# falfab/orb_slam_cuda

Measured on AMD Instinct MI355X. Metric: frames/s ORB extract+match, 1241×376 mono nFeatures=2000; achieved HBM GB/s, higher is better.
Workload: dtype u8

## Files before the change

orb_slam_cuda_amd/csrc/orbx_host.hip:

```cpp
#include <hip/hip_runtime.h>

#include <algorithm>
#include <atomic>
#include <chrono>
#include <condition_variable>
#include <cfloat>
#include <cstdarg>
#include <climits>
#include <cmath>
#include <cstdio>
#include <cstdlib>
#include <cstring>
#include <mutex>
#include <string>
#include <thread>
#include <vector>

#include "orbx_internal.h"
#include "orbx_sincosf.h"

namespace orbx {

__global__ __launch_bounds__(256) void copy2d_kernel(uint8_t* __restrict__ d, size_t dp, const uint8_t* __restrict__ s,
                                                     size_t sp, size_t w, size_t rows) {
// ... 12 lines not shown
size_t quadtree_lds_bytes(const ExtractParams& P);
size_t quadtree_legacy_lds_bytes(const ExtractParams& P);
size_t quadtree_sorted_lds_bytes(const ExtractParams& P, int big);
int quadtree_sorted_ownmax(const ExtractParams& P, int big, size_t budget);
extern const void* quadtree_kernel_ptr(const ExtractParams& P);
size_t pyr_band_lds_bytes(const ExtractParams& P);
void blur_strip_dims(int small, int* strip, int* rows);
extern const void* pyr_band_kernel_ptr();
extern int pyr_band_occupancy(size_t lds);
}

using namespace orbx;

static size_t out_desc_off(int cap_frame) { return (16 + (size_t)cap_frame * sizeof(orbx_kp) + 15) & ~(size_t)15; }

static thread_local std::string g_err;
static int fail(int code, const char* fmt, ...) {
  char buf[512];
  va_list ap;
  va_start(ap, fmt);
  vsnprintf(buf, sizeof buf, fmt, ap);
  va_end(ap);
  g_err = buf;
  return code;
}
#define HIP_OK(expr)                                                                        \
  do {                                                                                      \
    hipError_t e_ = (expr);                                                                 \
    if (e_ != hipSuccess) return fail(ORBX_EDEVICE, "%s: %s", #expr, hipGetErrorString(e_)); \
  } while (0)

namespace {

inline int cv_round(float v) { return (int)lrintf(v); }
inline int cv_floor(float v) { int i = (int)v; return i - (i > v); }
inline short sat_short(int v) { return (short)std::min(std::max(v, (int)SHRT_MIN), (int)SHRT_MAX); }

struct DeviceBuf {
  void* p = nullptr;
  size_t n = 0;
  ~DeviceBuf() { if (p) (void)hipFree(p); }
  int alloc(size_t bytes) {
    if (p) { (void)hipFree(p); p = nullptr; }
    n = bytes;
    if (!bytes) return ORBX_OK;
    if (hipMalloc(&p, bytes) != hipSuccess) return fail(ORBX_ENOMEM, "hipMalloc(%zu) failed", bytes);
    return ORBX_OK;
  }
  template <class T> T* as() const { return (T*)p; }
};

struct Plan {
  int W = 0, H = 0, B = 0;
  ExtractParams P{};
  std::vector<CellGeom> cells;
  std::vector<int2> rtab;
  DeviceBuf pyr, blur, rtab_d, cells_d, umax_d, slots, cell_counts, qkeys, qcounts, qties, qscratch, qnscratch,
      err;
};

}

struct orbx_extractor {
  orbx_config cfg{};
  std::vector<float> scale, inv_scale, sigma2, inv_sigma2;
  std::vector<int> nfeat;
  int umax[16];
  Plan plan;
  hipStream_t stream = nullptr;
  DeviceBuf d_in, d_out;
  void* h_in = nullptr;
  void* h_out = nullptr;
  size_t h_in_bytes = 0, h_out_bytes = 0;
  hipGraphExec_t graph = nullptr;
  int graph_w = 0, graph_h = 0;
  bool graph_hp = false;
  bool last_single = false;
  bool last_empty = false;
  int warm_w = 0, warm_h = 0;
  int last_batch = 0;
  const uint8_t* last_frames = nullptr;
  size_t last_fpitch = 0, last_rstride = 0;
  bool timing = false;
  hipEvent_t ev[6] = {};
  void* user_ev[ORBX_STAGE_EVENTS] = {};
  bool has_user_ev = false;
  WsOrder ws;
  bool host_pyr = false;
  bool host_pyr_valid = false;
  void* h_pyr = nullptr;
  size_t h_pyr_bytes = 0;
  long long h_pyr_off[kMaxLevels] = {};
  hipStream_t pstream = nullptr;
  hipEvent_t pev[2] = {};
  DeviceBuf d_depth;
  void* h_depth = nullptr;
  void* h_tail = nullptr;
  size_t h_depth_bytes = 0, h_tail_bytes = 0;
  hipStream_t dstream = nullptr;
  hipEvent_t dev = nullptr;
  std::vector<float> prof_t[4];
  char order[6] = {};
  std::mutex mu;
};

WsOrder* orbx::extractor_ws(orbx_handle h) { return h ? &h->ws : nullptr; }
// ... 87 lines not shown
    const int b0 = sat_short(cv_round((1.f - fy) * 2048)), b1 = sat_short(cv_round(fy * 2048));
    yt[dy] = make_int2(clip(sy, 0, sh) | (clip(sy + 1, 0, sh) << 16), (b0 & 0xFFFF) | (b1 << 16));
  }
}

struct PyrCols {
  int nct = 1;
  std::vector<int> lo, chi, ohi;
  int lpitch[kMaxLevels] = {};
};

static bool plan_pyr_cols(const ExtractParams& P, const std::vector<int2>& rtab, int nct, PyrCols& C) {
  const int L = P.L, WL = P.lv[L - 1].w;
  if (nct > 1 && WL / nct < 32) return false;
  C.nct = nct;
  C.lo.assign((size_t)nct * L, 0);
  C.chi.assign((size_t)nct * L, 0);
  C.ohi.assign((size_t)nct * L, 0);
  auto src_lo_x = [&](int l, int x) { return rtab[P.lv[l].xtab2 + std::min(x, P.lv[l].w - 1)].x; };
  auto src_hi_x = [&](int l, int x) { return rtab[P.lv[l].xtab2 + std::min(x, P.lv[l].w - 1)].x + 1; };
  for (int c = 0; c < nct; ++c) {
    C.lo[c * L + L - 1] = c == 0 ? 0 : ((int)((long long)c * WL / nct) & ~1);
    C.chi[c * L + L - 1] = C.ohi[c * L + L - 1] = (c + 1 < nct ? ((int)((long long)(c + 1) * WL / nct) & ~1) : WL) - 1;
  }
  for (int l = L - 2; l >= 0; --l)
    for (int c = 0; c < nct; ++c) C.lo[c * L + l] = c == 0 ? 0 : (src_lo_x(l + 1, C.lo[c * L + l + 1]) & ~1);
  for (int l = L - 2; l >= 0; --l)
    for (int c = 0; c < nct; ++c) {
      const int own_hi = c + 1 < nct ? C.lo[(c + 1) * L + l] - 1 : P.lv[l].w - 1;
      if (own_hi < C.lo[c * L + l]) return false;
      C.ohi[c * L + l] = own_hi;
      C.chi[c * L + l] = std::max(src_hi_x(l + 1, C.chi[c * L + l + 1]), l > 0 ? own_hi : 0);
    }
  for (int l = 0; l < L; ++l) {
    int p = 0;
    for (int c = 0; c < nct; ++c) {
      const int lo = C.lo[c * L + l], hi = C.chi[c * L + l];
      p = std::max(p, l == 0 ? ((hi - (lo & ~15) + 1 + 15) & ~15) : ((hi - lo + 1 + 8 + 15) & ~15));
    }
    if (const char* e = getenv("ORBX_PYR_PADMOD")) {
      const int m = (l == 0 ? atoi(e) & ~15 : atoi(e)) % 128, step = l == 0 ? 16 : 4;
      while (p % 128 != m) p += step;
    }
    C.lpitch[l] = p;
  }
  for (int l = 1; l < L; ++l) {
    if (C.lpitch[l - 1] % 4) return false;
    for (int c = 0; c < nct; ++c)
      if (C.chi[c * L + l] - C.lo[c * L + l] + 1 > 8 * 512) return false;
  }
  return true;
}

static void plan_band_pyramid(ExtractParams& P, std::vector<int2>& rtab) {
  P.pyr_fused = 0;
  const int L = P.L;
  if (L < 2) return;
  auto src_lo = [&](int l, int y) { return P.lv[l].area2x ? 2 * y : (rtab[P.lv[l].ytab + y].x & 0xFFFF); };
  auto src_hi = [&](int l, int y) { return P.lv[l].area2x ? 2 * y + 1 : (rtab[P.lv[l].ytab + y].x >> 16); };
  const int HL = P.lv[L - 1].h;
  const size_t budgets[2] = {78 * 1024, 160 * 1024 - 1024};
  const int R0 = std::max(1, (HL + 17) / 18);
  struct Cand {
    int R, nb, nct;
    size_t need0, need1, ybytes;
    long long cost;
    std::vector<int> lo, chi, ohi;
    PyrCols cols;
  };
  std::vector<Cand> cands;
  PyrCols colplans[3];
  bool colok[3];
  for (int k = 0; k < 3; ++k) colok[k] = plan_pyr_cols(P, rtab, 1 << k, colplans[k]);
  const int Rmax = std::max(R0 + 5, (HL + 3) / 4);
  for (int R = Rmax; R >= std::max(1, R0 / 3); --R) {
    const int nb = (HL + R - 1) / R;
    if (!cands.empty() && cands.back().nb == nb) continue;
    std::vector<int> lo((size_t)nb * L), chi((size_t)nb * L), ohi((size_t)nb * L);
    for (int b = 0; b < nb; ++b) {
      lo[b * L + L - 1] = b * R;
      chi[b * L + L - 1] = ohi[b * L + L - 1] = std::min((b + 1) * R, HL) - 1;
    }
    for (int l = L - 2; l >= 0; --l)
      for (int b = 0; b < nb; ++b) lo[b * L + l] = b == 0 ? 0 : src_lo(l + 1, lo[b * L + l + 1]);
    for (int l = L - 2; l >= 0; --l)
      for (int b = 0; b < nb; ++b) {
        const int own_hi = b + 1 < nb ? lo[(b + 1) * L + l] - 1 : P.lv[l].h - 1;
        ohi[b * L + l] = own_hi;
        chi[b * L + l] = std::max(src_hi(l + 1, chi[b * L + l + 1]), l > 0 ? own_hi : 0);
      }
    size_t ybytes = 0;
    for (int b = 0; b < nb; ++b) {
      size_t s = 0;
      for (int l = 1; l < L; ++l) s += (size_t)(chi[b * L + l] - lo[b * L + l] + 1) * 8;
      ybytes = std::max(ybytes, s);
    }
    for (int k = 0; k < 3; ++k) {
      if (!colok[k]) continue;
      const PyrCols& C = colplans[k];
      size_t need[2] = {0, 0};
      for (int l = 0; l < L; ++l) {
        int rows = 0;
        for (int b = 0; b < nb; ++b) rows = std::max(rows, chi[b * L + l] - lo[b * L + l] + 1);
        need[l & 1] = std::max(need[l & 1], (size_t)rows * C.lpitch[l]);
      }
      need[0] = (need[0] + 15) & ~(size_t)15;
// ... 16 lines not shown
  if (ek) {
    for (const char* p = ek; *p && keep.size() < 8;) {
      int nb = 0, nct = 0, used = 0;
      if (sscanf(p, "%d:%d%n", &nb, &nct, &used) != 2) break;
      for (int i = 0; i < (int)cands.size(); ++i)
        if (cands[i].nb == nb && cands[i].nct == nct) keep.push_back(i);
      p += used;
      if (*p == ',') ++p;
    }
  }
  if (keep.empty()) {
    int def = -1;
    for (int i = 0; i < (int)cands.size(); ++i)
      if (cands[i].nct == 1 && cands[i].need0 + cands[i].need1 + cands[i].ybytes + 16 <= budgets[0] &&
          (def < 0 || std::abs(cands[i].nb - (HL + R0 - 1) / R0) < std::abs(cands[def].nb - (HL + R0 - 1) / R0)))
        def = i;
    if (def < 0) def = 0;
    keep.push_back(def);
    std::vector<ExtractParams::PyrPlan> sim(cands.size());
    for (size_t i = 0; i < cands.size(); ++i) {
      sim[i].nbands = cands[i].nb;
      sim[i].nct = cands[i].nct;
      sim[i].cost = (int)cands[i].cost;
      sim[i].occ = cands[i].need0 + cands[i].need1 + cands[i].ybytes + 16 <= budgets[0] ? 2 : 1;
    }
    const int batches[8] = {1, 2, 4, 8, 16, 32, 64, P.B};
    for (int bt : batches) {
      const int best = pick_pyr_plan(sim.data(), (int)sim.size(), bt, 256);
      if (keep.size() < 8 && std::find(keep.begin(), keep.end(), best) == keep.end()) keep.push_back(best);
    }
    for (int d = 1; keep.size() < 8 && d < (int)cands.size(); ++d)
      for (int i : {def - d, def + d})
        if (i >= 0 && i < (int)cands.size() && cands[i].nct == 1 && keep.size() < 8 &&
            std::find(keep.begin(), keep.end(), i) == keep.end())
          keep.push_back(i);
  }
  P.pyr_nplans = 0;
  for (int i : keep) {
    const Cand& c = cands[i];
    ExtractParams::PyrPlan& q = P.pyr_plan[P.pyr_nplans++];
    q.nbands = c.nb;
    q.nct = c.nct;
    q.lds_a = (int)c.need0;
    q.lds_b = (int)c.need1;
    q.lds_y = (int)c.ybytes;
    q.cost = (int)c.cost;
    q.occ = 0;
    q.bands = (int)rtab.size();
    for (int b = 0; b < c.nb; ++b)
      for (int l = 0; l < L; ++l) {
        rtab.push_back(make_int2(c.lo[b * L + l], c.chi[b * L + l]));
        rtab.push_back(make_int2(c.lo[b * L + l], c.ohi[b * L + l]));
      }
    q.ctiles = (int)rtab.size();
    const PyrCols& C = c.cols;
    for (int t = 0; t < C.nct; ++t)
      for (int l = 0; l < L; ++l) {
        const int lo = C.lo[t * L + l];
        rtab.push_back(make_int2(lo, C.chi[t * L + l]));
        rtab.push_back(make_int2(lo, C.ohi[t * L + l]));
        rtab.push_back(make_int2(C.lpitch[l], l == 0 ? (lo & ~15) : lo));
      }
  }
  P.pyr_fused = 1;
  select_pyr_plan(P, 0);
}

static bool qt_code_tables(const LevelGeom& g, std::vector<uint32_t>& t, int* bits) {
  int R = 0;
  while ((1 << R) < g.nIni) ++R;
  if (R > 5 || g.boxW < 1 || g.boxH < 1 || g.boxW > 0xFFFF || g.boxH > 0xFFFF) return false;
  const int Dh = (13 - R) / 2;
  t.assign((size_t)g.boxW + g.boxH, 0u);
  for (int x = 0; x < g.boxW; ++x) {
    const int r = std::min((int)((float)x / g.hX), g.nIni - 1);
    int a = (int)(g.hX * (float)r), c = (int)(g.hX * (float)(r + 1));
    uint32_t code = (uint32_t)r << (2 * Dh);
    for (int j = 0; j < Dh; ++j) {
      const int mid = a + (int)std::ceil((float)(c - a) / 2.f);
      const int bit = x >= mid;
      if (bit) a = mid; else c = mid;
      code |= (uint32_t)bit << (2 * (Dh - 1 - j));
    }
    t[x] = code;
  }
  for (int y = 0; y < g.boxH; ++y) {
    int a = 0, c = g.boxH;
    uint32_t code = 0;
    for (int j = 0; j < Dh; ++j) {
      const int mid = a + (int)std::ceil((float)(c - a) / 2.f);
      const int bit = y >= mid;
      if (bit) a = mid; else c = mid;
      code |= (uint32_t)bit << (2 * (Dh - 1 - j) + 1);
    }
    t[(size_t)g.boxW + y] = code;
  }
  *bits = (Dh << 8) | ((R + 2 * Dh) << 16);
  return true;
}

static int build_plan(orbx_extractor* h, int W, int Hh, int B) {
  Plan& pl = h->plan;
  const orbx_config& c = h->cfg;
  const int L = c.nlevels;
  ExtractParams P{};
  P.L = L;
  P.B = B;
  const int ini = std::min(std::max(c.ini_th_fast, 0), 255), mn = std::min(std::max(c.min_th_fast, 0), 255);
  P.t_ini = ini;
  P.t_min = mn;
  P.t_low = std::min(ini, mn);
  P.pattern_upstream = c.pattern_mode == ORBX_PATTERN_UPSTREAM;
  gaussian7(P.gauss);
  pl.cells.clear();
  pl.rtab.clear();
  long long lvl_off = 0;
  int slot = 0, kbase = 0, maxnodes = 0, maxcells = 0;
  for (int l = 0; l < L; ++l) {
    LevelGeom& g = P.lv[l];
    const float inv = h->inv_scale[l];
    g.w = cv_round((float)W * inv);
    g.h = cv_round((float)Hh * inv);
    if (g.w > kMaxLevelDim || g.h > kMaxLevelDim)
      return fail(ORBX_EINVAL, "level %d is %dx%d; at most %d px per side", l, g.w, g.h, kMaxLevelDim);
    g.pitch = (g.w + 63) & ~63;
    g.plane = (long long)g.h * g.pitch;
    g.minBX = kEdgeThreshold - 3;
    g.minBY = g.minBX;
    g.maxBX = g.w - kEdgeThreshold + 3;
    g.maxBY = g.h - kEdgeThreshold + 3;
    const float width = (float)(g.maxBX - g.minBX), height = (float)(g.maxBY - g.minBY);
    g.nCols = (int)(width / kGridW);
    g.nRows = (int)(height / kGridW);
    if (g.nCols < 1 || g.nRows < 1)
      return fail(ORBX_EINVAL,
                  "level %d (%dx%d) is smaller than one %d-px FAST cell inside the %d-px border; "
                  "the reference divides by zero here (src/ORBextractor.cc:1144-1147)",
                  l, g.w, g.h, kGridW, kEdgeThreshold);
    g.wCell = (int)std::ceil(width / g.nCols);
    g.hCell = (int)std::ceil(height / g.nRows);
    if (g.wCell + 6 > kMaxRoi - 1 || g.hCell + 6 > kMaxRoi - 1)
      return fail(ORBX_EINVAL, "level %d cell %dx%d exceeds the ROI tile", l, g.wCell, g.hCell);
    g.cell0 = (int)pl.cells.size();
    g.slot0 = slot;
    for (int i = 0; i < g.nRows; i++) {
      const float iniY = g.minBY + i * g.hCell;
      float maxY = iniY + g.hCell + 6;
      const bool skipRow = iniY >= g.maxBY - 3;
      if (maxY > g.maxBY) maxY = g.maxBY;
      for (int j = 0; j < g.nCols; j++) {
        const float iniX = g.minBX + j * g.wCell;
        float maxX = iniX + g.wCell + 6;
        const bool skip = skipRow || iniX >= g.maxBX - 6;
        if (maxX > g.maxBX) maxX = g.maxBX;
// ... 103 lines not shown
      if (d * (unsigned long long)B * e < (1ull << 32)) P.blur_magic[v] = (unsigned)m;
    }
  }
  if (maxnodes > 65000) return fail(ORBX_EINVAL, "nfeatures too large for the quadtree node table");
  P.slots_per_frame = slot;
  P.ncells_total = (int)pl.cells.size();
  {
    const unsigned long long d = (unsigned long long)P.ncells_total;
    P.ncells_magic = 0u;
    if (d > 1) {
      const unsigned long long m = ((1ull << 32) + d - 1) / d, e = m * d - (1ull << 32);
      if (d * (unsigned long long)B * e < (1ull << 32)) P.ncells_magic = (unsigned)m;
    }
  }
  P.kp_per_frame = kbase;
  P.maxnodes = maxnodes;
  int sn = 1;
  while (sn < maxnodes) sn <<= 1;
  P.sortn = sn;
  P.max_cells_level = maxcells;
  P.kcap_lds = 0;
  {
    const char* e = getenv("ORBX_QT_GENERIC");
    P.qt_lean = maxnodes < 16384 && !(e && e[0] == '1');
    const char* so = getenv("ORBX_QT_SORTED");
    P.qt_sorted = P.qt_lean && P.qt_nbmax > 0 && !(so && so[0] == '0');
  }
  {
#ifndef ORBX_QT_LDS_KB
#define ORBX_QT_LDS_KB 80
#endif
    const size_t base = quadtree_legacy_lds_bytes(P);
    size_t small = ORBX_QT_LDS_KB * 1024, big = 160 * 1024 - 512;
    if (const char* e = getenv("ORBX_QT_LDS_KB")) small = (size_t)std::max(32, atoi(e)) * 1024;
    P.qt_big = base + 16 * 1024 > small ? 1 : 0;
    const size_t budget = P.qt_big ? big : small;
    P.kcap_lds = base < budget ? (int)((budget - base) / 6) & ~15 : 0;
    if (P.qt_sorted) {
      P.qt_ownmax = quadtree_sorted_ownmax(P, P.qt_big, budget);
      if (!P.qt_ownmax || quadtree_sorted_lds_bytes(P, P.qt_big) > budget) P.qt_sorted = 0;
    }
    if (maxnodes > 2 * (P.qt_big ? 1024 : kQtThreads)) P.qt_sorted = 0;
    if (getenv("ORBX_PLAN_INFO"))
      fprintf(stderr,
              "plan %dx%d B %d: quadtree LDS legacy %zu sorted %zu (budget %zu) sorted %d big %d maxnodes %d "
              "nbmax %d tabmax %d ownmax %d\n",
              W, Hh, B, base, P.qt_nbmax ? quadtree_sorted_lds_bytes(P, P.qt_big) : (size_t)0, budget, P.qt_sorted,
              P.qt_big, maxnodes, P.qt_nbmax, P.qt_tabmax, P.qt_ownmax);
  }
  pl.P = P;
  pl.W = W;
  pl.H = Hh;
  pl.B = B;
  int rc;
  if ((rc = pl.pyr.alloc((size_t)lvl_off))) return rc;
  if ((rc = pl.blur.alloc((size_t)lvl_off))) return rc;
  if ((rc = pl.rtab_d.alloc(std::max<size_t>(pl.rtab.size(), 1) * sizeof(int2)))) return rc;
  if ((rc = pl.cells_d.alloc(pl.cells.size() * sizeof(CellGeom)))) return rc;
  if ((rc = pl.umax_d.alloc(16 * sizeof(int)))) return rc;
  if ((rc = pl.slots.alloc((size_t)B * slot * 4 + 4 + 4 * 96))) return rc;
  if ((rc = pl.cell_counts.alloc((size_t)B * P.ncells_total * 4))) return rc;
  if ((rc = pl.qkeys.alloc((size_t)B * P.kp_per_frame * 4))) return rc;
  if ((rc = pl.qcounts.alloc((size_t)B * L * 4 + 4 * kMaxLevels))) return rc;
  if ((rc = pl.qties.alloc((size_t)B * L * 16))) return rc;
  if ((rc = pl.qscratch.alloc((size_t)B * slot * 4 + 4))) return rc;
  if ((rc = pl.qnscratch.alloc((size_t)B * slot * 2 + 4))) return rc;
  if ((rc = pl.err.alloc(16))) return rc;
  HIP_OK(hipMemcpy(pl.rtab_d.p, pl.rtab.data(), pl.rtab.size() * sizeof(int2), hipMemcpyHostToDevice));
  HIP_OK(hipMemcpy(pl.cells_d.p, pl.cells.data(), pl.cells.size() * sizeof(CellGeom), hipMemcpyHostToDevice));
  HIP_OK(hipMemcpy(pl.umax_d.p, h->umax, 16 * sizeof(int), hipMemcpyHostToDevice));
  HIP_OK(hipMemset(pl.err.p, 0, 16));
  if (P.pyr_fused && getenv("ORBX_PYR_PROF") && getenv("ORBX_PYR_PROF")[0] == '1')
    for (int i = 0; i < P.pyr_nplans; ++i)
      fprintf(stderr, "pyr plan %d: %d bands x %d column tiles, lds %d + %d + %d, cost %d\n", i,
              P.pyr_plan[i].nbands, P.pyr_plan[i].nct, P.pyr_plan[i].lds_a, P.pyr_plan[i].lds_b, P.pyr_plan[i].lds_y,
              P.pyr_plan[i].cost);
  if (P.pyr_fused) {
    size_t mx = 0;
    for (int i = 0; i < P.pyr_nplans; ++i) {
      ExtractParams Q = P;
      select_pyr_plan(Q, i);
      mx = std::max(mx, pyr_band_lds_bytes(Q));
    }
    if (raise_lds_limit(pyr_band_kernel_ptr(), mx))
      return fail(ORBX_EDEVICE, "LDS limit of pyr_band_kernel: %s", hipGetErrorString(hipGetLastError()));
    for (int i = 0; i < P.pyr_nplans; ++i) {
      ExtractParams Q = P;
      select_pyr_plan(Q, i);
      pl.P.pyr_plan[i].occ = pyr_band_occupancy(pyr_band_lds_bytes(Q));
      if (getenv("ORBX_PYR_PROF") && getenv("ORBX_PYR_PROF")[0] == '1')
        fprintf(stderr, "pyr plan %d: %d workgroups per CU\n", i, pl.P.pyr_plan[i].occ);
    }
  }
  if (raise_lds_limit(quadtree_kernel_ptr(P), quadtree_lds_bytes(P)))
    return fail(ORBX_EDEVICE, "LDS limit of quadtree_kernel: %s", hipGetErrorString(hipGetLastError()));
  return ORBX_OK;
}

static ExtractBuffers buffers_of(const Plan& pl) {
  ExtractBuffers X;
  X.pyr = pl.pyr.as<uint8_t>();
  X.blur = pl.blur.as<uint8_t>();
  X.rtab = pl.rtab_d.as<int2>();
  X.cells = pl.cells_d.as<CellGeom>();
  X.umax = pl.umax_d.as<int>();
  X.slots = pl.slots.as<uint32_t>();
  X.cell_counts = pl.cell_counts.as<int>();
// ... 113 lines not shown
  orbx_extractor* h = new orbx_extractor();
  h->cfg = c;
  memcpy(h->order, extract_stage_order(), 6);
  compute_scales(h);
  h->plan.B = c.max_batch;
  int rc = deferred ? ORBX_OK : build_plan(h, c.width, c.height, c.max_batch);
  if (rc) { delete h; return rc; }
  const char* t = getenv("ORBX_TIMING");
  h->timing = t && t[0] == '1';
  if (h->timing)
    for (auto& e : h->ev) (void)hipEventCreate(&e);
  *out = h;
  return ORBX_OK;
}

int orbx_destroy(orbx_handle h) {
  if (!h) return ORBX_OK;
  (void)hipSetDevice(h->cfg.device);
  if (h->stream) (void)hipStreamSynchronize(h->stream);
  for (auto& e : h->ev)
    if (e) (void)hipEventDestroy(e);
  if (h->ws.ev) (void)hipEventSynchronize(h->ws.ev);
  h->ws.release();
  if (h->graph) (void)hipGraphExecDestroy(h->graph);
  if (h->pstream) (void)hipStreamSynchronize(h->pstream);
  if (h->prof_t[0].size() > 20) {
    double med[4];
    for (int k = 0; k < 4; ++k) {
      std::vector<float> v(h->prof_t[k].begin() + 20, h->prof_t[k].end());
      std::nth_element(v.begin(), v.begin() + v.size() / 2, v.end());
      med[k] = v[v.size() / 2] * 1e6;
    }
    fprintf(stderr, "orbx_extract host phases, median of %zu calls (us): stage %.1f issue %.1f wait %.1f out %.1f\n",
            h->prof_t[0].size() - 20, med[0], med[1], med[2], med[3]);
  }
  if (h->h_in) (void)hipHostFree(h->h_in);
  if (h->h_out) (void)hipHostFree(h->h_out);
  if (h->h_pyr) (void)hipHostFree(h->h_pyr);
  if (h->dstream) (void)hipStreamSynchronize(h->dstream);
  if (h->h_depth) (void)hipHostFree(h->h_depth);
  if (h->h_tail) (void)hipHostFree(h->h_tail);
  if (h->dev) (void)hipEventDestroy(h->dev);
  if (h->dstream) (void)hipStreamDestroy(h->dstream);
  for (auto& e : h->pev)
    if (e) (void)hipEventDestroy(e);
  if (h->pstream) (void)hipStreamDestroy(h->pstream);
  if (h->stream) (void)hipStreamDestroy(h->stream);
  delete h;
  return ORBX_OK;
}

int orbx_frame_capacity(orbx_handle h) { return h ? h->plan.P.kp_per_frame : 0; }

int orbx_extract_batch(orbx_handle h, const uint8_t* d_frames, int batch, size_t frame_pitch, size_t row_stride,
                       orbx_kp* d_kps, uint8_t* d_desc, int* d_counts, void* stream) {
  if (!h || !d_frames || !d_kps || !d_desc || !d_counts) return fail(ORBX_EINVAL, "null argument");
  std::lock_guard<std::mutex> lk(h->mu);
  if (batch < 1 || batch > h->plan.B) return fail(ORBX_EINVAL, "batch %d not in 1..max_batch(%d)", batch, h->plan.B);
  if (h->plan.W == 0)
    return fail(ORBX_EINVAL, "no frame size yet: the handle was created with width/height 0 and has seen no orbx_extract");
  if (row_stride < (size_t)h->plan.W) return fail(ORBX_EINVAL, "row_stride < width");
  HIP_OK(hipSetDevice(h->cfg.device));
  void** ev = h->has_user_ev ? h->user_ev : (h->timing ? (void**)h->ev : nullptr);
  h->has_user_ev = false;
  if (h->ws.before((hipStream_t)stream)) return fail(ORBX_EDEVICE, "stream wait on the handle's last use failed");
  const int rc = launch_extract(h->plan.P, buffers_of(h->plan), d_frames, batch, frame_pitch, row_stride, d_kps,
                                d_desc, d_counts, stream, ev, nullptr, nullptr, h->order);
  if (!rc && h->ws.after((hipStream_t)stream)) return fail(ORBX_EDEVICE, "event record failed");
  h->last_batch = batch;
  h->last_frames = d_frames;
  h->last_fpitch = frame_pitch;
  h->last_rstride = row_stride;
  h->host_pyr_valid = false;
  h->last_single = false;
  h->last_empty = false;
  if (rc) return fail(rc, "kernel launch failed: %s", hipGetErrorString(hipGetLastError()));
  return ORBX_OK;
}

static int host_reserve(void** p, size_t* have, size_t need) {
  if (*have >= need) return ORBX_OK;
  if (*p) (void)hipHostFree(*p);
  *p = nullptr;
  *have = 0;
  if (hipHostMalloc(p, need, hipHostMallocDefault) != hipSuccess) return fail(ORBX_ENOMEM, "hipHostMalloc(%zu)", need);
  *have = need;
  return ORBX_OK;
}


static size_t host_pyr_layout(orbx_extractor* h) {
  const ExtractParams& P = h->plan.P;
  size_t off = 0;
  for (int l = 1; l < P.L; ++l) {
    h->h_pyr_off[l] = (long long)off;
    off += (size_t)P.lv[l].plane;
  }
  return off;
}

static int issue_one_frame(orbx_extractor* h, size_t pitch, int hh, int cap_frame) {
  hipStream_t s = h->stream;
  const ExtractParams& P = h->plan.P;
  HIP_OK(hipMemcpyAsync(h->d_in.p, h->h_in, pitch * hh, hipMemcpyHostToDevice, s));
  uint8_t* d = h->d_out.as<uint8_t>();
  const size_t doff = out_desc_off(cap_frame);
// ... 745 lines not shown
```

orb_slam_cuda_amd/csrc/orbx_pyramid.hip:

```cpp
#include <cstdio>
#include <cstdlib>
#include <vector>

#include "orbx_device.cuh"

namespace orbx {

constexpr int kPyrTW = 256, kPyrTH = 16;
constexpr int kPyrMaxSrcW = 576;
constexpr int kPyrMaxSrcH = 36;

__global__ __launch_bounds__(256) void pyr_resize_kernel(
    const uint8_t* __restrict__ src, long long src_fs, int src_pitch, int sw, int sh, uint8_t* __restrict__ dst,
    long long dst_fs, int dst_pitch, int dw, int dh, const int2* __restrict__ xtab, const int2* __restrict__ ytab,
    int xmax, int area2x, int src_aligned16) {
  __shared__ __attribute__((aligned(16))) uint8_t tile[kPyrMaxSrcH][kPyrMaxSrcW];
  __shared__ int2 s_xt[kPyrTW];
  __shared__ int2 s_yt[kPyrTH];
  const int wg = xcd_remap(blockIdx.x + gridDim.x * (blockIdx.y + gridDim.y * blockIdx.z),
                           gridDim.x * gridDim.y * gridDim.z);
  const int f = wg / (gridDim.x * gridDim.y), tid = threadIdx.x;
  const int x0 = (wg % gridDim.x) * kPyrTW, y0 = ((wg / gridDim.x) % gridDim.y) * kPyrTH;
  const int nx = min(kPyrTW, dw - x0), ny = min(kPyrTH, dh - y0);
  const uint8_t* S = src + f * src_fs;
// ... 36 lines not shown
  __syncthreads();
  const int cx = (tid & 63) * 4, ry = (tid >> 6) * 4;
  if (cx >= nx) return;
  int sxl[4], a0v[4], a1v[4], rep[4];
#pragma unroll
  for (int q = 0; q < 4; ++q) {
    const int c = min(cx + q, nx - 1);
    const int2 xt = s_xt[c];
    sxl[q] = xt.x - a0;
    a0v[q] = (short)(xt.y & 0xFFFF);
    a1v[q] = (short)(xt.y >> 16);
    rep[q] = area2x ? 0 : (x0 + c >= xmax);
  }
  uint8_t* D = dst + f * dst_fs + (long long)(y0 + ry) * dst_pitch + x0 + cx;
#pragma unroll
  for (int rr = 0; rr < 4; ++rr) {
    if (ry + rr >= ny) break;
    const int2 yt = s_yt[ry + rr];
    const uint8_t* r0 = tile[(yt.x & 0xFFFF) - sy_lo];
    const uint8_t* r1 = tile[(yt.x >> 16) - sy_lo];
    int v[4];
#pragma unroll
    for (int q = 0; q < 4; ++q) {
      const int s = sxl[q];
      if (area2x) {
        v[q] = (r0[s] + r0[s + 1] + r1[s] + r1[s + 1] + 2) >> 2;
      } else {
        int D0, D1;
        if (!rep[q]) {
          D0 = __mul24((int)r0[s], a0v[q]) + __mul24((int)r0[s + 1], a1v[q]);
          D1 = __mul24((int)r1[s], a0v[q]) + __mul24((int)r1[s + 1], a1v[q]);
        } else {
          D0 = r0[s] * 2048;
          D1 = r1[s] * 2048;
        }
        const int b0 = (short)(yt.y & 0xFFFF), b1 = (short)(yt.y >> 16);
        v[q] = sat_u8((__mul24(D0, b0) + __mul24(D1, b1) + (1 << 21)) >> 22);
      }
    }
    const uint32_t packed = pack4_u8(v[0], v[1], v[2], v[3]);
    uint8_t* drow = D + (long long)rr * dst_pitch;
    if (cx + 4 <= nx) {
      *(uint32_t*)drow = packed;
    } else {
      for (int q = 0; cx + q < nx; ++q) drow[q] = (uint8_t)(packed >> (8 * q));
    }
  }
}

#ifndef ORBX_PYR_THREADS
#define ORBX_PYR_THREADS 512
#endif
constexpr int kPyrBandThreads = ORBX_PYR_THREADS;
constexpr uint32_t kPyrAreaA = 2048u | (2048u << 16);
constexpr int kPyrAreaB4 = 2048 | (2048 << 16);
#ifndef ORBX_PYR_WPE
#define ORBX_PYR_WPE 5
#endif

__device__ __forceinline__ int pyr_col(int gi, int G, int q) { return 2 * (gi + (q >> 1) * G) + (q & 1); }

typedef unsigned short pyr_us2_t __attribute__((ext_vector_type(2)));

__device__ __forceinline__ int band_div(int i, float rcp) { return (int)(((float)i + 0.5f) * rcp); }

struct BandCols {
  int off[4];
  uint32_t sel[8];
  uint32_t a01[8];
};
__device__ __forceinline__ void band_load(const uint8_t* row, const BandCols& bc, uint32_t (&p)[8]) {
#pragma unroll
  for (int k = 0; k < 4; ++k) {
    const uint32_t* d = (const uint32_t*)(row + bc.off[k]);
    p[2 * k] = d[0];
    p[2 * k + 1] = d[1];
  }
}
__device__ __forceinline__ void band_hpass(const uint32_t (&p)[8], const BandCols& bc, uint32_t (&D)[8]) {
#pragma unroll
  for (int q = 0; q < 8; ++q) {
    const uint32_t pp = __builtin_amdgcn_perm(p[q | 1], p[q & ~1], bc.sel[q]);
    D[q] = __builtin_amdgcn_udot2(__builtin_bit_cast(pyr_us2_t, pp), __builtin_bit_cast(pyr_us2_t, bc.a01[q]), 0u, false);
  }
}

__device__ __forceinline__ uint32_t band_mad24(uint32_t a, uint32_t b, uint32_t c) {
  uint32_t d;
  asm("v_mad_u32_u24 %0, %1, %2, %3" : "=v"(d) : "v"(a), "v"(b), "v"(c));
  return d;
}

struct BandRowCtx {
  const uint8_t* src;
  uint8_t* dst;
  uint8_t* g[4];
  const int2* yt;
  int spitch, dpitch, gpitch, src_lo, row0;
  unsigned own_lo, own_n;
  bool st2[4], st1[4], any1;
};
__device__ __forceinline__ void band_row(const BandRowCtx& c, int r, uint32_t loff, uint32_t goff, int& have,
                                         const BandCols& bc, int G, uint32_t (&Da)[8], uint32_t (&Db)[8]) {
  const int2 yt = c.yt[r - c.row0];
  const int y0 = yt.x & 0xFFFF, y1 = yt.x >> 16;
  const uint8_t* const row1 = c.src + __mul24(y1 - c.src_lo, c.spitch);
  uint32_t p1[8];
  if (y0 != have) {
    uint32_t p0[8];
    band_load(c.src + __mul24(y0 - c.src_lo, c.spitch), bc, p0);
    band_load(row1, bc, p1);
    band_hpass(p0, bc, Da);
  } else {
    band_load(row1, bc, p1);
  }
  band_hpass(p1, bc, Db);
  have = y1;
  const uint32_t b0 = (uint32_t)yt.y & 0xFFFFu, b1 = (uint32_t)yt.y >> 16;
  const bool owned = (unsigned)r - c.own_lo < c.own_n;
  uint32_t pk[4];
#pragma unroll
  for (int k = 0; k < 4; ++k) {
    const uint32_t va = band_mad24(Da[2 * k], b0, band_mad24(Db[2 * k], b1, 1u << 23));
    const uint32_t vb = band_mad24(Da[2 * k + 1], b0, band_mad24(Db[2 * k + 1], b1, 1u << 23));
    pk[k] = __builtin_amdgcn_perm(vb, va, 0x0c0c0703u);
    *(uint16_t*)(c.dst + loff + 2 * k * G) = (uint16_t)pk[k];
    if (owned && c.st2[k]) *(uint16_t*)(c.g[k] + goff) = (uint16_t)pk[k];
  }
  if (c.any1 && owned) {
#pragma unroll
    for (int k = 0; k < 4; ++k)
      if (c.st1[k]) c.g[k][goff] = (uint8_t)pk[k];
  }
}

__global__ __launch_bounds__(kPyrBandThreads) __attribute__((amdgpu_waves_per_eu(ORBX_PYR_WPE))) void pyr_band_kernel(ExtractParams P, LevelPtrs lp,
                                                                   const int2* __restrict__ rtab, int* dbg) {
  extern __shared__ __attribute__((aligned(16))) uint8_t smem[];
  const unsigned long long t_begin = __builtin_amdgcn_s_memtime();
  const int nb = P.pyr_nbands, nct = P.pyr_nct, L = P.L, tid = threadIdx.x;
  const int wg = xcd_remap(blockIdx.x, gridDim.x);
  const int f = wg / (nb * nct), tile = wg - f * (nb * nct), band = tile / nct, ct = tile - band * nct;
  const int2* bt = rtab + P.pyr_bands + (long long)band * L * 2;
  const int2* xt = rtab + P.pyr_ctiles + (long long)ct * L * 3;
  uint8_t* const bufA = smem;
  uint8_t* const bufB = smem + P.pyr_lds_a;
  int2* const s_yt = (int2*)(smem + P.pyr_lds_a + P.pyr_lds_b);
  int yrow = 0, ytot = 0, yarea = 1, ytab = 0;
#pragma unroll
  for (int l = 1; l < kMaxLevels; ++l) {
    const int2 cd = bt[2 * min(l, L - 1)];
    const int n = l < L ? cd.y - cd.x + 1 : 0;
    if (tid >= ytot && tid < ytot + n) {
      yrow = cd.x + tid - ytot;
      yarea = P.lv[l].area2x;
      ytab = P.lv[l].ytab;
    }
    ytot += n;
  }
  auto y_entry = [&](int area, int tab, int r) {
    if (area) return make_int2((2 * r) | ((2 * r + 1) << 16), kPyrAreaB4);
    const int2 e = rtab[tab + r];
    return make_int2(e.x, e.y << 2);
  };
  int2 yval = make_int2(0, 0);
  if (tid < ytot) yval = y_entry(yarea, ytab, yrow);
  for (int i = tid + kPyrBandThreads; i < ytot; i += kPyrBandThreads) {
    int rem = i;
    for (int l = 1; l < L; ++l) {
      const int2 cd = bt[2 * l];
      const int n = cd.y - cd.x + 1;
      if (rem < n) {
        const LevelGeom& g = P.lv[l];
        const int r = cd.x + rem;
        s_yt[i] = y_entry(g.area2x, g.ytab, r);
        break;
      }
      rem -= n;
    }
  }

  {
    const int2 c0 = bt[0], x0c = xt[0], x0p = xt[2];
    const int rows = c0.y - c0.x + 1, lp0 = x0p.x, org = x0p.y, pitch = lp.pitch[0];
    const int xe = min(x0c.y, P.lv[0].w - 1);
    const uint8_t* S = lp.base[0] + f * lp.fstride[0] + (long long)c0.x * pitch + org;
    if (lp.aligned16[0]) {
      typedef unsigned int u32x4 __attribute__((ext_vector_type(4)));
      const int nch = ((xe - org) >> 4) + 1, total = rows * nch;
      const float rnch = __builtin_amdgcn_rcpf((float)nch);
      for (int i0 = tid; i0 < total; i0 += 4 * kPyrBandThreads) {
        u32x4 v[4];
        int so[4], lo[4];
#pragma unroll
        for (int q = 0; q < 4; ++q) {
          const int i = min(i0 + q * kPyrBandThreads, total - 1);
          const int r = band_div(i, rnch), ch = i - r * nch;
          lo[q] = r * pitch + ch * 16;
          so[q] = r * lp0 + ch * 16;
        }
#pragma unroll
        for (int q = 0; q < 4; ++q) v[q] = *(const u32x4*)(S + lo[q]);
        if (i0 == tid && tid < ytot) s_yt[tid] = yval;
#pragma unroll
        for (int q = 0; q < 4; ++q) *(u32x4*)(bufA + so[q]) = v[q];
      }
      if (tid >= total && tid < ytot) s_yt[tid] = yval;
    } else {
      if (tid < ytot) s_yt[tid] = yval;
      const int ncol = xe - org + 1;
      for (int r = 0; r < rows; ++r)
        for (int c = tid; c < ncol; c += kPyrBandThreads) bufA[r * lp0 + c] = S[(long long)r * pitch + c];
    }
  }

  int2 nxt[8];
  int nxt_gi = 0, nxt_ra = 0, nxt_rb = -1;
  auto fetch_cols = [&](int l) {
    const LevelGeom& g = P.lv[l];
    const int2 xc = xt[3 * l];
    const int G = (xc.y - xc.x + 1 + 7) >> 3;
    const float rG = __builtin_amdgcn_rcpf((float)G);
    const int chunk = band_div(tid, rG), gi = tid - chunk * G;
    const int2 cd = bt[2 * l];
    const int nrows = cd.y - cd.x + 1, nchunks = band_div(kPyrBandThreads, rG);
    const int len = band_div(nrows, __builtin_amdgcn_rcpf((float)nchunks)), rem = nrows - len * nchunks;
    nxt_gi = gi;
    nxt_ra = cd.x + chunk * len + min(chunk, rem);
    nxt_rb = chunk < nchunks ? nxt_ra + len - (chunk < rem ? 0 : 1) : nxt_ra - 1;
#pragma unroll
    for (int q = 0; q < 8; ++q) nxt[q] = rtab[g.xtab2 + min(xc.x + pyr_col(gi, G, q), g.w - 1)];
  };
  fetch_cols(1);
  lds_sync();
  if (dbg && tid == 0) dbg[blockIdx.x * 16] = (int)(__builtin_amdgcn_s_memtime() - t_begin);

  int yoff = 0;
  for (int l = 1; l < L; ++l) {
    const LevelGeom& g = P.lv[l];
    const int2 cs = bt[2 * (l - 1)], cd = bt[2 * l], own = bt[2 * l + 1];
    const int2 xc = xt[3 * l], xo = xt[3 * l + 1], sp = xt[3 * (l - 1) + 2], dp = xt[3 * l + 2];
    const int G = (xc.y - xc.x + 1 + 7) >> 3, gi = nxt_gi, ra = nxt_ra, rb = nxt_rb;
    BandCols bc;
#pragma unroll
    for (int q = 0; q < 8; ++q) {
      const int sx = nxt[q].x - sp.y;
      if (!(q & 1)) bc.off[q >> 1] = sx & ~3;
      const uint32_t o = (uint32_t)(sx - bc.off[q >> 1]);
      bc.sel[q] = 0x0c000c00u | o | ((o + 1) << 16);
      bc.a01[q] = g.area2x ? kPyrAreaA : (uint32_t)nxt[q].y;
    }
    if (l + 1 < L) fetch_cols(l + 1);
    BandRowCtx c;
    c.src = (l & 1) ? bufA : bufB;
    c.dst = (l & 1) ? bufB : bufA;
    c.yt = s_yt + yoff;
    c.spitch = sp.x, c.dpitch = dp.x, c.gpitch = lp.pitch[l], c.src_lo = cs.x, c.row0 = cd.x;
    c.own_lo = (unsigned)own.x, c.own_n = (unsigned)(own.y - own.x + 1);
#pragma unroll
    for (int k = 0; k < 4; ++k) {
      const int gx = xc.x + 2 * (gi + k * G);
      c.g[k] = (uint8_t*)lp.base[l] + f * lp.fstride[l] + xc.x + 2 * k * G;
      c.st2[k] = gx >= xo.x && gx < xo.y;
      c.st1[k] = gx == xo.y;
    }
    c.any1 = c.st1[0] | c.st1[1] | c.st1[2] | c.st1[3];
    uint32_t loff = (uint32_t)(__mul24(ra - cd.x, c.dpitch) + 2 * gi);
    uint32_t goff = (uint32_t)(ra * c.gpitch + 2 * gi);
    uint32_t Da[8], Db[8];
    int have = -1;
    for (int r = ra; r <= rb; r += 2) {
      band_row(c, r, loff, goff, have, bc, G, Da, Db);
      loff += c.dpitch, goff += c.gpitch;
      if (r + 1 <= rb) band_row(c, r + 1, loff, goff, have, bc, G, Db, Da);
      loff += c.dpitch, goff += c.gpitch;
    }
    yoff += cd.y - cd.x + 1;
    lds_sync();
    if (dbg && tid == 0) dbg[blockIdx.x * 16 + l] = (int)(__builtin_amdgcn_s_memtime() - t_begin);
  }
}

size_t pyr_band_lds_bytes(const ExtractParams& P) { return (size_t)P.pyr_lds_a + P.pyr_lds_b + P.pyr_lds_y + 16; }
const void* pyr_band_kernel_ptr() { return (const void*)pyr_band_kernel; }
int pyr_band_occupancy(size_t lds) {
  int n = 0;
  if (hipOccupancyMaxActiveBlocksPerMultiprocessor(&n, pyr_band_kernel, kPyrBandThreads, lds) != hipSuccess) return 1;
  return std::max(1, n);
}

static int launch_band(const ExtractParams& P, const LevelPtrs& lp, const int2* rtab, int batch, hipStream_t s) {
  static int* dbg = nullptr;
  static int dbg_cap = 0;
  static const bool prof = getenv("ORBX_PYR_PROF") && getenv("ORBX_PYR_PROF")[0] == '1';
  const int nwg = P.pyr_nbands * P.pyr_nct * batch;
  if (prof && nwg > dbg_cap) {
    if (dbg) (void)hipFree(dbg);
    (void)hipMalloc(&dbg, (size_t)nwg * 16 * 4);
    dbg_cap = nwg;
  }
  hipLaunchKernelGGL(pyr_band_kernel, dim3(nwg), dim3(kPyrBandThreads), pyr_band_lds_bytes(P), s, P, lp, rtab,
                     prof ? dbg : nullptr);
  if (prof) {
    std::vector<int> h((size_t)nwg * 16);
    (void)hipStreamSynchronize(s);
    (void)hipMemcpy(h.data(), dbg, h.size() * 4, hipMemcpyDeviceToHost);
    double avg[16] = {0};
    int mx[16] = {0};
    for (int w = 0; w < nwg; ++w)
      for (int k = 0; k < P.L; ++k) {
        avg[k] += h[w * 16 + k];
        mx[k] = std::max(mx[k], h[w * 16 + k]);
      }
    fprintf(stderr, "pyr_band plans (bands x tiles/cost/lds):");
    for (int i = 0; i < P.pyr_nplans; ++i)
      fprintf(stderr, " %dx%d/%d/%d", P.pyr_plan[i].nbands, P.pyr_plan[i].nct, P.pyr_plan[i].cost,
              P.pyr_plan[i].lds_a + P.pyr_plan[i].lds_b + P.pyr_plan[i].lds_y + 16);
    fprintf(stderr, "\n");
    fprintf(stderr, "pyr_band: %d WGs (%d bands x %d tiles); phase cycles avg/max:", nwg, P.pyr_nbands, P.pyr_nct);
// ... 36 lines not shown
```

Before: 195,400.

## Precompute pyramid band row tables and per-column records on host

The fused band-pyramid kernel no longer derives its per-row y-table entries and per-column gather offsets, byte-select masks, weights and store flags on every launch. These are now built once at plan time into rtab, along with a host-side validator and a test entry point. The kernel loads them as packed 16-byte vectors, cutting index arithmetic and scattered rtab lookups from its prologue and level loop. In exchange the table grows and each column tile carries a fourth entry per level, and plans whose records fail validation are dropped.

New measurement: 199,200, median of 6. 1.02x the previous value.

```diff
diff --git a/orb_slam_cuda_amd/csrc/orbx_host.hip b/orb_slam_cuda_amd/csrc/orbx_host.hip
--- a/orb_slam_cuda_amd/csrc/orbx_host.hip
+++ b/orb_slam_cuda_amd/csrc/orbx_host.hip
@@ -88,6 +88,7 @@
 
 struct Plan {
   int W = 0, H = 0, B = 0;
+  long long level_bytes = 0;
   ExtractParams P{};
   std::vector<CellGeom> cells;
   std::vector<int2> rtab;
@@ -281,6 +282,43 @@
   return true;
 }
 
+static long long pyr_records_ok(const ExtractParams& P, const std::vector<int2>& rtab,
+                                const ExtractParams::PyrPlan& q) {
+  const int L = P.L;
+  long long n = 0;
+  for (int b = 0; b < q.nbands; ++b) {
+    const int2* bt = rtab.data() + q.bands + (long long)b * L * 2;
+    long long rows = 0;
+    for (int l = 1; l < L; ++l) rows += bt[2 * l].y - bt[2 * l].x + 1;
+    const int2 yh = bt[1];
+    if (yh.x <= 0 || yh.y != rows || (long long)yh.x + yh.y > (long long)rtab.size() || rows * 8 > q.lds_y) return -1;
+  }
+  for (int t = 0; t < q.nct; ++t)
+    for (int l = 1; l < L; ++l) {
+      const int2* xt = rtab.data() + q.ctiles + ((long long)t * L + l) * 4;
+      const int2 xc = xt[0], xo = xt[1], sp = xt[-4 + 2];
+      const int G = (xc.y - xc.x + 1 + 7) >> 3;
+      const long long at = xt[3].x;
+      if (at <= 0 || (at & 1) || at + 12LL * G > (long long)rtab.size()) return -1;
+      if (xo.x < 0 || xo.y >= P.lv[l].w || xo.x > xo.y) return -1;
+      for (int gi = 0; gi < G; ++gi, ++n) {
+        const uint32_t* rec = (const uint32_t*)(rtab.data() + at + 12LL * gi);
+        for (int k = 0; k < 4; ++k) {
+          const int off = (int)rec[k], gx = xc.x + 2 * (gi + k * G);
+          if (off < 0 || (off & 3) || off > sp.x + 8) return -1;
+          for (int j = 0; j < 2; ++j) {
+            const uint32_t sel = rec[4 + 2 * k + j], o = sel & 0xFF;
+            if (sel != (0x0c000c00u | o | ((o + 1) << 16)) || o > 6) return -1;
+          }
+          if (((rec[20] >> k) & 1) && (gx < xo.x || gx + 1 > xo.y)) return -1;
+          if (((rec[20] >> (4 + k)) & 1) && gx != xo.y) return -1;
+        }
+        if (rec[20] >> 8) return -1;
+      }
+    }
+  return n;
+}
+
 static void plan_band_pyramid(ExtractParams& P, std::vector<int2>& rtab) {
   P.pyr_fused = 0;
   const int L = P.L;
@@ -403,16 +441,56 @@
         rtab.push_back(make_int2(c.lo[b * L + l], c.chi[b * L + l]));
         rtab.push_back(make_int2(c.lo[b * L + l], c.ohi[b * L + l]));
       }
+    for (int b = 0; b < c.nb; ++b) {
+      const int at = (int)rtab.size();
+      for (int l = 1; l < L; ++l)
+        for (int r = c.lo[b * L + l]; r <= c.chi[b * L + l]; ++r) {
+          const int2 e = rtab[P.lv[l].ytab + r];
+          rtab.push_back(P.lv[l].area2x ? make_int2((2 * r) | ((2 * r + 1) << 16), 2048 | (2048 << 16))
+                                        : make_int2(e.x, e.y << 2));
+        }
+      rtab[q.bands + b * L * 2 + 1] = make_int2(at, (int)rtab.size() - at);
+    }
     q.ctiles = (int)rtab.size();
     const PyrCols& C = c.cols;
+    auto origin = [&](int t, int l) { return l == 0 ? (C.lo[t * L] & ~15) : C.lo[t * L + l]; };
     for (int t = 0; t < C.nct; ++t)
       for (int l = 0; l < L; ++l) {
         const int lo = C.lo[t * L + l];
         rtab.push_back(make_int2(lo, C.chi[t * L + l]));
         rtab.push_back(make_int2(lo, C.ohi[t * L + l]));
-        rtab.push_back(make_int2(C.lpitch[l], l == 0 ? (lo & ~15) : lo));
+        rtab.push_back(make_int2(C.lpitch[l], origin(t, l)));
+        rtab.push_back(make_int2(0, 0));
       }
-  }
+    for (int t = 0; t < C.nct; ++t)
+      for (int l = 1; l < L; ++l) {
+        if (rtab.size() & 1) rtab.push_back(make_int2(0, 0));
+        rtab[q.ctiles + (t * L + l) * 4 + 3].x = (int)rtab.size();
+        const LevelGeom& g = P.lv[l];
+        const int lo = C.lo[t * L + l], ohi = C.ohi[t * L + l];
+        const int G = (C.chi[t * L + l] - lo + 1 + 7) >> 3, org = origin(t, l - 1);
+        for (int gi = 0; gi < G; ++gi) {
+          uint32_t rec[24] = {};
+          for (int qq = 0; qq < 8; ++qq) {
+            const int col = lo + 2 * (gi + (qq >> 1) * G) + (qq & 1);
+            const int2 e = rtab[g.xtab2 + std::min(col, g.w - 1)];
+            const int sx = e.x - org;
+            if (!(qq & 1)) rec[qq >> 1] = (uint32_t)(sx & ~3);
+            const uint32_t o = (uint32_t)sx - rec[qq >> 1];
+            rec[4 + qq] = 0x0c000c00u | o | ((o + 1) << 16);
+            rec[12 + qq] = g.area2x ? (2048u | (2048u << 16)) : (uint32_t)e.y;
+          }
+          for (int k = 0; k < 4; ++k) {
+            const int gx = lo + 2 * (gi + k * G);
+            if (gx >= lo && gx < ohi) rec[20] |= 1u << k;
+            if (gx == ohi) rec[20] |= 16u << k;
+          }
+          for (int i = 0; i < 24; i += 2) rtab.push_back(make_int2((int)rec[i], (int)rec[i + 1]));
+        }
+      }
+    if (pyr_records_ok(P, rtab, q) < 0) --P.pyr_nplans;
+  }
+  if (!P.pyr_nplans) return;
   P.pyr_fused = 1;
   select_pyr_plan(P, 0);
 }
@@ -450,7 +528,7 @@
   return true;
 }
 
-static int build_plan(orbx_extractor* h, int W, int Hh, int B) {
+static int build_plan_host(orbx_extractor* h, int W, int Hh, int B) {
   Plan& pl = h->plan;
   const orbx_config& c = h->cfg;
   const int L = c.nlevels;
@@ -660,7 +738,17 @@
   pl.W = W;
   pl.H = Hh;
   pl.B = B;
+  pl.level_bytes = lvl_off;
+  return ORBX_OK;
+}
+
+static int build_plan(orbx_extractor* h, int W, int Hh, int B) {
   int rc;
+  if ((rc = build_plan_host(h, W, Hh, B))) return rc;
+  Plan& pl = h->plan;
+  const ExtractParams& P = pl.P;
+  const int L = P.L, slot = P.slots_per_frame;
+  const long long lvl_off = pl.level_bytes;
   if ((rc = pl.pyr.alloc((size_t)lvl_off))) return rc;
   if ((rc = pl.blur.alloc((size_t)lvl_off))) return rc;
   if ((rc = pl.rtab_d.alloc(std::max<size_t>(pl.rtab.size(), 1) * sizeof(int2)))) return rc;
@@ -880,6 +968,24 @@
 
 int orbx_frame_capacity(orbx_handle h) { return h ? h->plan.P.kp_per_frame : 0; }
 
+int orbx_pyr_plan_check(const orbx_config* cfg, long long* records, int cap, int* nplans) {
+  if (!cfg || !records || !nplans) return fail(ORBX_EINVAL, "null argument");
+  if (cfg->nlevels < 1 || cfg->nlevels > kMaxLevels || !(cfg->scale_factor > 1.0f) || cfg->width <= 0 ||
+      cfg->height <= 0 || cfg->max_batch < 1)
+    return fail(ORBX_EINVAL, "bad configuration");
+  orbx_extractor* h = new orbx_extractor();
+  h->cfg = *cfg;
+  compute_scales(h);
+  const int rc = build_plan_host(h, cfg->width, cfg->height, cfg->max_batch);
+  if (!rc) {
+    const ExtractParams& P = h->plan.P;
+    *nplans = P.pyr_fused ? P.pyr_nplans : 0;
+    for (int i = 0; i < *nplans && i < cap; ++i) records[i] = pyr_records_ok(P, h->plan.rtab, P.pyr_plan[i]);
+  }
+  delete h;
+  return rc;
+}
+
 int orbx_extract_batch(orbx_handle h, const uint8_t* d_frames, int batch, size_t frame_pitch, size_t row_stride,
                        orbx_kp* d_kps, uint8_t* d_desc, int* d_counts, void* stream) {
   if (!h || !d_frames || !d_kps || !d_desc || !d_counts) return fail(ORBX_EINVAL, "null argument");
diff --git a/orb_slam_cuda_amd/csrc/orbx_pyramid.hip b/orb_slam_cuda_amd/csrc/orbx_pyramid.hip
--- a/orb_slam_cuda_amd/csrc/orbx_pyramid.hip
+++ b/orb_slam_cuda_amd/csrc/orbx_pyramid.hip
@@ -112,8 +112,6 @@
 #define ORBX_PYR_THREADS 512
 #endif
 constexpr int kPyrBandThreads = ORBX_PYR_THREADS;
-constexpr uint32_t kPyrAreaA = 2048u | (2048u << 16);
-constexpr int kPyrAreaB4 = 2048 | (2048 << 16);
 #ifndef ORBX_PYR_WPE
 #define ORBX_PYR_WPE 5
 #endif
@@ -194,6 +192,10 @@
   }
 }
 
+#if (defined(ORBX_PYR_NOSTAGE) || defined(ORBX_PYR_STAGE_NOLDS)) && !defined(ORBX_DIAG)
+#error "result-changing diagnostic switches need -DORBX_DIAG (tools/variant.sh)"
+#endif
+
 __global__ __launch_bounds__(kPyrBandThreads) __attribute__((amdgpu_waves_per_eu(ORBX_PYR_WPE))) void pyr_band_kernel(ExtractParams P, LevelPtrs lp,
                                                                    const int2* __restrict__ rtab, int* dbg) {
   extern __shared__ __attribute__((aligned(16))) uint8_t smem[];
@@ -202,43 +204,15 @@
   const int wg = xcd_remap(blockIdx.x, gridDim.x);
   const int f = wg / (nb * nct), tile = wg - f * (nb * nct), band = tile / nct, ct = tile - band * nct;
   const int2* bt = rtab + P.pyr_bands + (long long)band * L * 2;
-  const int2* xt = rtab + P.pyr_ctiles + (long long)ct * L * 3;
+  const int2* xt = rtab + P.pyr_ctiles + (long long)ct * L * 4;
   uint8_t* const bufA = smem;
   uint8_t* const bufB = smem + P.pyr_lds_a;
   int2* const s_yt = (int2*)(smem + P.pyr_lds_a + P.pyr_lds_b);
-  int yrow = 0, ytot = 0, yarea = 1, ytab = 0;
-#pragma unroll
-  for (int l = 1; l < kMaxLevels; ++l) {
-    const int2 cd = bt[2 * min(l, L - 1)];
-    const int n = l < L ? cd.y - cd.x + 1 : 0;
-    if (tid >= ytot && tid < ytot + n) {
-      yrow = cd.x + tid - ytot;
-      yarea = P.lv[l].area2x;
-      ytab = P.lv[l].ytab;
-    }
-    ytot += n;
-  }
-  auto y_entry = [&](int area, int tab, int r) {
-    if (area) return make_int2((2 * r) | ((2 * r + 1) << 16), kPyrAreaB4);
-    const int2 e = rtab[tab + r];
-    return make_int2(e.x, e.y << 2);
-  };
+  const int2 yh = bt[1];
+  const int ytot = yh.y;
   int2 yval = make_int2(0, 0);
-  if (tid < ytot) yval = y_entry(yarea, ytab, yrow);
-  for (int i = tid + kPyrBandThreads; i < ytot; i += kPyrBandThreads) {
-    int rem = i;
-    for (int l = 1; l < L; ++l) {
-      const int2 cd = bt[2 * l];
-      const int n = cd.y - cd.x + 1;
-      if (rem < n) {
-        const LevelGeom& g = P.lv[l];
-        const int r = cd.x + rem;
-        s_yt[i] = y_entry(g.area2x, g.ytab, r);
-        break;
-      }
-      rem -= n;
-    }
-  }
+  if (tid < ytot) yval = rtab[yh.x + tid];
+  for (int i = tid + kPyrBandThreads; i < ytot; i += kPyrBandThreads) s_yt[i] = rtab[yh.x + i];
 
   {
     const int2 c0 = bt[0], x0c = xt[0], x0p = xt[2];
@@ -249,7 +223,11 @@
       typedef unsigned int u32x4 __attribute__((ext_vector_type(4)));
       const int nch = ((xe - org) >> 4) + 1, total = rows * nch;
       const float rnch = __builtin_amdgcn_rcpf((float)nch);
+#ifdef ORBX_PYR_NOSTAGE
+      for (int i0 = tid; i0 < 0; i0 += 4 * kPyrBandThreads) {
+#else
       for (int i0 = tid; i0 < total; i0 += 4 * kPyrBandThreads) {
+#endif
         u32x4 v[4];
         int so[4], lo[4];
 #pragma unroll
@@ -262,10 +240,19 @@
 #pragma unroll
         for (int q = 0; q < 4; ++q) v[q] = *(const u32x4*)(S + lo[q]);
         if (i0 == tid && tid < ytot) s_yt[tid] = yval;
+#ifdef ORBX_PYR_STAGE_NOLDS
+#pragma unroll
+        for (int q = 0; q < 4; ++q) asm volatile("" ::"v"(v[q]));
+#else
 #pragma unroll
         for (int q = 0; q < 4; ++q) *(u32x4*)(bufA + so[q]) = v[q];
+#endif
       }
+#ifdef ORBX_PYR_NOSTAGE
+      if (tid < ytot) s_yt[tid] = yval;
+#else
       if (tid >= total && tid < ytot) s_yt[tid] = yval;
+#endif
     } else {
       if (tid < ytot) s_yt[tid] = yval;
       const int ncol = xe - org + 1;
@@ -274,11 +261,12 @@
     }
   }
 
-  int2 nxt[8];
+  typedef unsigned int rec4_t __attribute__((ext_vector_type(4)));
+  rec4_t nxt[5];
+  uint32_t nxt_flags = 0;
   int nxt_gi = 0, nxt_ra = 0, nxt_rb = -1;
   auto fetch_cols = [&](int l) {
-    const LevelGeom& g = P.lv[l];
-    const int2 xc = xt[3 * l];
+    const int2 xc = xt[4 * l];
     const int G = (xc.y - xc.x + 1 + 7) >> 3;
     const float rG = __builtin_amdgcn_rcpf((float)G);
     const int chunk = band_div(tid, rG), gi = tid - chunk * G;
@@ -288,8 +276,10 @@
     nxt_gi = gi;
     nxt_ra = cd.x + chunk * len + min(chunk, rem);
     nxt_rb = chunk < nchunks ? nxt_ra + len - (chunk < rem ? 0 : 1) : nxt_ra - 1;
-#pragma unroll
-    for (int q = 0; q < 8; ++q) nxt[q] = rtab[g.xtab2 + min(xc.x + pyr_col(gi, G, q), g.w - 1)];
+    const rec4_t* rec = (const rec4_t*)(rtab + xt[4 * l + 3].x) + __mul24(gi, 6);
+#pragma unroll
+    for (int i = 0; i < 5; ++i) nxt[i] = rec[i];
+    nxt_flags = ((const uint32_t*)rec)[20];
   };
   fetch_cols(1);
   lds_sync();
@@ -297,19 +287,17 @@
 
   int yoff = 0;
   for (int l = 1; l < L; ++l) {
-    const LevelGeom& g = P.lv[l];
     const int2 cs = bt[2 * (l - 1)], cd = bt[2 * l], own = bt[2 * l + 1];
-    const int2 xc = xt[3 * l], xo = xt[3 * l + 1], sp = xt[3 * (l - 1) + 2], dp = xt[3 * l + 2];
+    const int2 xc = xt[4 * l], sp = xt[4 * (l - 1) + 2], dp = xt[4 * l + 2];
     const int G = (xc.y - xc.x + 1 + 7) >> 3, gi = nxt_gi, ra = nxt_ra, rb = nxt_rb;
     BandCols bc;
 #pragma unroll
-    for (int q = 0; q < 8; ++q) {
-      const int sx = nxt[q].x - sp.y;
-      if (!(q & 1)) bc.off[q >> 1] = sx & ~3;
-      const uint32_t o = (uint32_t)(sx - bc.off[q >> 1]);
-      bc.sel[q] = 0x0c000c00u | o | ((o + 1) << 16);
-      bc.a01[q] = g.area2x ? kPyrAreaA : (uint32_t)nxt[q].y;
-    }
+    for (int q = 0; q < 4; ++q) {
+      bc.off[q] = (int)nxt[0][q];
+      bc.sel[q] = nxt[1][q], bc.sel[4 + q] = nxt[2][q];
+      bc.a01[q] = nxt[3][q], bc.a01[4 + q] = nxt[4][q];
+    }
+    const uint32_t flags = nxt_flags;
     if (l + 1 < L) fetch_cols(l + 1);
     BandRowCtx c;
     c.src = (l & 1) ? bufA : bufB;
@@ -319,12 +307,11 @@
     c.own_lo = (unsigned)own.x, c.own_n = (unsigned)(own.y - own.x + 1);
 #pragma unroll
     for (int k = 0; k < 4; ++k) {
-      const int gx = xc.x + 2 * (gi + k * G);
       c.g[k] = (uint8_t*)lp.base[l] + f * lp.fstride[l] + xc.x + 2 * k * G;
-      c.st2[k] = gx >= xo.x && gx < xo.y;
-      c.st1[k] = gx == xo.y;
-    }
-    c.any1 = c.st1[0] | c.st1[1] | c.st1[2] | c.st1[3];
+      c.st2[k] = (flags >> k) & 1u;
+      c.st1[k] = (flags >> (4 + k)) & 1u;
+    }
+    c.any1 = (flags & 0xF0u) != 0;
     uint32_t loff = (uint32_t)(__mul24(ra - cd.x, c.dpitch) + 2 * gi);
     uint32_t goff = (uint32_t)(ra * c.gpitch + 2 * gi);
     uint32_t Da[8], Db[8];
```
